# numericalEFT/MCIntegration.jl

Hardware: AMD Instinct MI355X
Metric: Msamples/sec (whole node), 16-D Gaussian :vegas (higher is better)
Workload: dtype f64

## Files before the change

### mcintegration.jl_amd/_lib.py

```python
import ctypes as C
import os

_PKG = os.path.dirname(os.path.abspath(__file__))
_SO = os.path.join(_PKG, "lib", "libmci_hip.so")

MCI_OK = 0
ERR_NAMES = {1: "INVALID", 2: "HIP", 3: "COMPILE", 4: "NORMALIZATION", 5: "HISTOGRAM", 6: "COMM", 7: "NO_DEVICE"}
CONTINUOUS, DISCRETE, FERMIK = 0, 1, 2
VEGAS, VEGASMC, MCMC = 0, 1, 2
ABI_VERSION = 5
SOLVERS = {"vegas": VEGAS, "vegasmc": VEGASMC, "mcmc": MCMC, VEGAS: VEGAS, VEGASMC: VEGASMC, MCMC: MCMC}

c_double_p = C.POINTER(C.c_double)
c_int32_p = C.POINTER(C.c_int32)


class MCIError(RuntimeError):
    def __init__(self, code, msg):
        super().__init__("[MCI_ERR_%s] %s" % (ERR_NAMES.get(code, code), msg))
        self.code = code


class LeafDesc(C.Structure):
    _fields_ = [("kind", C.c_int32), ("pool", C.c_int32), ("lower", C.c_double), ("upper", C.c_double),
# ... 107 lines not shown
    ("mci_last_chain_speculation", C.c_int, [_VP, c_int32_p, c_int32_p]),
    ("mci_chain_speculation_status", C.c_int, [_VP, C.c_int32, c_int32_p]),
    ("mci_vegas_check_status", C.c_int, [_VP, c_int32_p, c_int32_p]),
    ("mci_last_integrate_discarded", C.c_int, [_VP, C.POINTER(C.c_int64), c_int32_p]),
    ("mci_speculation_tree", C.c_int, [C.c_int32, C.c_double, C.c_int32, c_int32_p, c_int32_p, c_int32_p, C.POINTER(C.c_uint64), C.POINTER(C.c_uint64)]),
    ("mci_compile_chain_speculation", C.c_int, [_VP, C.c_int32]),
    ("mci_train", C.c_int, [_VP]),
    ("mci_sample_dump", C.c_int, [_VP, C.c_int32, C.c_uint64, C.c_int64, C.c_int64, C.c_int64, c_double_p, c_double_p, c_double_p]),
    ("mci_kernel_times_ms", C.c_int, [_VP, C.POINTER(C.c_float), C.c_int32, c_int32_p, c_int32_p, c_int32_p]),
    ("mci_kernel_clocks", C.c_int, [_VP, c_double_p, C.c_int32, c_int32_p]),
    ("mci_comm_times_ms", C.c_int, [_VP, C.POINTER(C.c_float), C.c_int32, c_int32_p]),
    ("mci_comm_collectives", C.c_int, [_VP, C.POINTER(C.c_int64), C.POINTER(C.c_int64)]),
    ("mci_reduce_size", C.c_int, [_VP, C.POINTER(C.c_int64)]),
    ("mci_external_reduce_done", C.c_int, [_VP]),
    ("mci_standardize_block", None, [C.c_int64, C.c_int64, C.c_int64, C.POINTER(C.c_int64), C.POINTER(C.c_int64)]),
    ("mci_chain_burnin", C.c_double, [C.c_int64, C.c_int64, C.c_int32]),
    ("mci_mcmc_burnin", C.c_int64, [C.c_int64, C.c_int64, C.c_int32, C.c_int32, C.c_int32, C.c_double]),
    ("mci_mcmc_auto_chains", C.c_int64, [C.c_int64, C.c_int64, C.c_int32, C.c_int32, C.c_int32, C.c_int64, C.c_int64, C.c_int32]),
    ("mci_get_hold_histogram", C.c_int, [_VP, C.POINTER(C.c_uint64)]),
    ("mci_mcmc_launch_valid", C.c_int, [_VP, c_int32_p, c_int32_p, C.POINTER(C.c_int64), C.POINTER(C.c_int64)]),
    ("mci_iteration_discard", C.c_int, [_VP]),
    ("mci_get_block_means", C.c_int, [_VP, C.c_int32, c_double_p, C.POINTER(C.c_int64), c_int32_p]),
    ("mci_reset_block_log", C.c_int, [_VP]),
    ("mci_lineage_sums", None, [c_double_p, C.c_int64, C.c_int64, C.c_int64, c_double_p, C.c_int64, C.c_int64, c_double_p, c_double_p]),
    ("mci_maxdof", None, [c_int32_p, C.c_int32, C.c_int32, c_int32_p]),
    ("mci_mean_std", None, [c_double_p, c_double_p, C.c_int64, C.c_int64, c_double_p, c_double_p]),
    ("mci_average", None, [c_double_p, c_double_p, C.c_int64, C.c_int64, C.c_int64, c_double_p, c_double_p, c_double_p]),
    ("mci_do_reweight", None, [c_double_p, c_double_p, C.c_int64, C.c_double, c_double_p]),
    ("mci_version", C.c_char_p, []),
    ("mci_abi_version", C.c_int32, []),
]
DEBUG_SIGNATURES = [
    ("mci_debug_persist_words", C.c_int, [_VP, C.POINTER(C.c_uint64), C.c_int32]),
    ("mci_debug_walk_counts", C.c_int, [_VP, C.POINTER(C.c_int64)]),
    ("mci_debug_plant_wrong_decision", C.c_int, [_VP, C.c_int32]),
    ("mci_debug_persist_spin_ticks", C.c_int, [_VP, C.c_uint64]),
    ("mci_debug_override", C.c_int, [C.c_char_p, C.c_int64, C.c_int32]),
    ("mci_debug_compiler_id", C.c_int, [C.c_char_p, C.c_char_p, C.c_int32]),
    ("mci_debug_split_chunks", C.c_int, [_VP, C.POINTER(C.c_int64), C.POINTER(C.c_int64)]),
    ("mci_debug_vegas_cursor", C.c_int, [_VP, C.POINTER(C.c_int32), C.POINTER(C.c_uint64)]),
    ("mci_debug_strat_d", C.c_int, [_VP, c_double_p, C.c_int64]),
    ("mci_debug_strat_start_d", C.c_int, [_VP, c_double_p, C.c_int64]),
    ("mci_debug_strat_dump", C.c_int, [_VP, C.c_int64, c_double_p, c_double_p, C.POINTER(C.c_int64), c_double_p, c_double_p]),
    ("mci_debug_mcmc_policy", C.c_int, [C.c_int64, C.c_int64, C.c_int64, C.c_int64]),
    ("mci_debug_vegas_check", C.c_int, [_VP, C.c_int32, C.c_uint64, C.c_int64, C.c_int64, C.c_int64, C.c_int64, c_double_p, c_double_p, c_double_p, c_double_p,
                                        C.POINTER(C.c_int64)]),
    ("mci_debug_vegas_check_launches", C.c_int, [_VP, C.POINTER(C.c_int64)]),
    ("mci_debug_vegas_check_layout", C.c_int, [_VP, c_int32_p, c_int32_p, c_double_p, C.POINTER(C.c_uint64), c_int32_p]),
    ("mci_debug_sweep_workgroups", C.c_int, [_VP, C.c_int32]),
    ("mci_debug_sweep_threads", C.c_int, [_VP, C.c_int32]),
    ("mci_debug_sweep_last_launch", C.c_int, [_VP, c_int32_p, c_int32_p]),
    ("mci_debug_sweep_lds_bytes", C.c_int, [_VP, C.POINTER(C.c_int64)]),
]

_lib = None


def library_path():
    return _SO


def use_rocm_compiler(rocm=None):
    root = rocm or os.environ.get("ROCM_PATH") or "/opt/rocm"
    mapped = set()
    try:
        with open("/proc/self/maps") as fh:
# ... 52 lines not shown
```

### mcintegration.jl_amd/csrc/mci_debug.h

```cpp
#ifndef MCI_DEBUG_H
#define MCI_DEBUG_H
#include "../../include/mci.h"
#ifdef __cplusplus
extern "C" {
#endif
int mci_debug_persist_words(mci_problem *prob, unsigned long long *out, int32_t n);
int mci_debug_walk_counts(mci_problem *prob, int64_t *out);
int mci_debug_plant_wrong_decision(mci_problem *prob, int32_t on);
int mci_debug_persist_spin_ticks(mci_problem *prob, unsigned long long ticks);
int mci_debug_override(const char *key, int64_t value, int32_t on);
int mci_debug_split_chunks(const mci_problem *prob, int64_t *chunks, int64_t *bytes);
int mci_debug_strat_dump(mci_problem *prob, int64_t n, double *x, double *y, int64_t *h, double *jac, double *w);
int mci_debug_strat_d(mci_problem *prob, double *d, int64_t n);
int mci_debug_strat_start_d(mci_problem *prob, double *d, int64_t n);
int mci_debug_vegas_cursor(const mci_problem *prob, int32_t *used, uint64_t *base);
int mci_debug_compiler_id(const char *set, char *out, int32_t n);
int mci_debug_mcmc_policy(int64_t pilot_steps, int64_t grow, int64_t carry_holds, int64_t carry_half_floors);
int mci_debug_vegas_check(mci_problem *prob, int32_t iteration, uint64_t seed, int64_t nevalperblock, int64_t block_lo, int64_t nblocks,
                          int64_t measurefreq, const double *x, const double *jac, const double *w, double *packed, int64_t *bad);
int mci_debug_vegas_check_launches(const mci_problem *prob, int64_t *launches);
int mci_debug_vegas_check_layout(const mci_problem *prob, int32_t *head, int32_t *draws, double *scales, uint64_t *own, int32_t *obs);
int mci_debug_sweep_workgroups(mci_problem *prob, int32_t g);
int mci_debug_sweep_threads(mci_problem *prob, int32_t threads);
int mci_debug_sweep_last_launch(const mci_problem *prob, int32_t *workgroups, int32_t *threads);
int mci_debug_sweep_lds_bytes(const mci_problem *prob, int64_t *bytes);
#ifdef __cplusplus
}
#endif
#endif
```

### mcintegration.jl_amd/csrc/mci_host_jit.h

```cpp
enum { kSlotVegasAny = 3, kSlotDump = 4, kSlotVegasmcSpec = 5, kSlotMcmcSpec = 6 };
static int kslot(int solver, int64_t measurefreq) { return solver == MCI_VEGAS && measurefreq != 1 ? kSlotVegasAny : solver; }
static int slot_solver(int slot) { return slot == kSlotVegasAny ? MCI_VEGAS : slot == kSlotVegasmcSpec ? MCI_VEGASMC : slot == kSlotMcmcSpec ? MCI_MCMC : slot; }

namespace {
struct Candidate {
    std::string src;
    int threads = 256;
    int unit = mcijit::kUnitSolver;
    std::vector<char> code;
    std::string log, path;
    bool cached = false;
    int rc = 0;
    long vgprs() const { return mcijit::kernel_vgprs(code, "mci_vegas_batch"); }
    long scratch() const { return mcijit::kernel_scratch_bytes(code, "mci_vegas_batch"); }
    int build(bool cache_only = false) { return rc = mcijit::compile(src, threads, code, log, cached, &path, unit, cache_only); }
    int failed(const std::string &of = "") const { return fail(MCI_ERR_COMPILE, "integrand failed to compile for gfx950%s:\n%s", of.c_str(), log.c_str()); }
};
void compile_all(const std::vector<Candidate *> &cs) {
    std::vector<std::thread> th;
    for (size_t i = 1; i < cs.size(); ++i) th.emplace_back([c = cs[i]] { c->build(); });
    if (!cs.empty()) cs[0]->build();
    for (auto &t : th) t.join();
}

// ... 484 lines not shown
    return MCI_OK;
}

int mci_set_iteration_counted(mci_problem *p, int32_t counted) {
    if (!p) return fail(MCI_ERR_INVALID, "NULL argument");
    p->launch_counted = counted != 0;
    return MCI_OK;
}

int mci_set_persistent(mci_problem *p, int32_t mode) {
    if (!p) return fail(MCI_ERR_INVALID, "NULL argument");
    if (mode < -1 || mode > 1) return fail(MCI_ERR_INVALID, "persistent mode must be -1 (automatic: launch-bound :vegas calls), 0 (one launch chain per iteration) or 1 (whenever the layout allows)");
    p->persistent = mode;
    return MCI_OK;
}

int mci_debug_persist_words(mci_problem *p, unsigned long long *out, int32_t n) {
    if (!p || !out || !p->d_persist) return fail(MCI_ERR_INVALID, "no persistent launch yet");
    HIPCHK(hipStreamSynchronize(p->ctx->stream));
    HIPCHK(hipMemcpy(out, p->d_persist, (size_t)(n < (int)kPersistWords ? n : (int)kPersistWords) * sizeof(unsigned long long), hipMemcpyDeviceToHost));
    return MCI_OK;
}

int mci_debug_walk_counts(mci_problem *p, int64_t *out) {
    if (!p || !out || !p->d_status) return fail(MCI_ERR_INVALID, "NULL argument");
    int h[2] = {0, 0};
    HIPCHK(hipStreamSynchronize(p->ctx->stream));
    HIPCHK(hipMemcpy(h, p->d_status + 1, sizeof(h), hipMemcpyDeviceToHost));
    out[0] = h[0];
    out[1] = h[1];
    return MCI_OK;
}

int mci_last_integrate_persistent(const mci_problem *p, int32_t *persistent) {
    if (!p || !persistent) return fail(MCI_ERR_INVALID, "NULL argument");
    *persistent = p->last_persistent ? 1 : 0;
    return MCI_OK;
}

int mci_last_chain_launch(const mci_problem *p, int64_t *nchain, int32_t *carried) {
    if (!p) return fail(MCI_ERR_INVALID, "NULL argument");
    if (nchain) *nchain = p->launch.last_nchain;
    if (carried) *carried = p->launch.last_carried ? 1 : 0;
    return MCI_OK;
}

int mci_check_status(mci_problem *p) {
    if (!p) return fail(MCI_ERR_INVALID, "NULL argument");
    if (p->ctx->offline) return fail(MCI_ERR_NO_DEVICE, "offline context");
    return check_status(p);
}
static int compile_persist(mci_problem *p, bool background);
static bool persist_layout_ok(const mci_problem *p);
static int compile_strat(mci_problem *p);
static int compile_sweep_unit(mci_problem *p, int which);
static bool sweep_leaves_unit(const mci_problem *p);
int mci_compile_solver(mci_problem *p, int32_t solver) {
    if (solver == MCI_VEGAS_PERSISTENT) {
        if (!persist_layout_ok(p)) return fail(MCI_ERR_INVALID, "this layout has no persistent :vegas kernel (mci_set_persistent)");
        return compile_persist(p, false);
    }
    if (solver == MCI_VEGASMC_LANES || solver == MCI_MCMC_LANES) return mci_compile_chain_speculation(p, solver == MCI_VEGASMC_LANES ? MCI_VEGASMC : MCI_MCMC);
    if (solver == MCI_VEGAS_STRAT) {
        if (!p->strat.on) return fail(MCI_ERR_INVALID, "the problem is not stratified (mci_set_stratification)");
        return compile_strat(p);
    }
// ... 51 lines not shown
```

### mcintegration.jl_amd/csrc/mci_host_problem.h

```cpp
int mci_problem_create(mci_ctx *ctx, const mci_problem_desc *d, mci_problem **out) {
    if (!ctx || !d || !out) return fail(MCI_ERR_INVALID, "NULL argument");
    if (d->nleaf < 1 || d->npool < 1 || d->nintegrand < 1) return fail(MCI_ERR_INVALID, "At least one integrand is required.");
    if (d->nintegrand > 31) return fail(MCI_ERR_INVALID, "at most 31 integrands are supported");
    mci_problem *p = new mci_problem();
    p->ctx = ctx;
    p->npool = d->npool;
    p->ni = d->nintegrand;
    const int Nd = p->ni + 1;
    p->dof.assign((size_t)Nd * p->npool, 0);
    for (int i = 0; i < p->ni * p->npool; ++i) {
        if (d->dof[i] < 0) { delete p; return fail(MCI_ERR_INVALID, "dof must be non-negative"); }
        p->dof[i] = d->dof[i];
    }
    p->maxdof.assign(p->npool, 0);
    mci_maxdof(p->dof.data(), Nd, p->npool, p->maxdof.data());
    p->pool_leaf0.assign(p->npool, -1);
    p->pool_nleaf.assign(p->npool, 0);
    auto &s = p->shape;
    int eoff = 0, aoff = 0, doff = 0, boff = 0;
    for (int l = 0; l < d->nleaf; ++l) {
        const mci_leaf_desc &ld = d->leaves[l];
        if (ld.pool < 0 || ld.pool >= p->npool) { delete p; return fail(MCI_ERR_INVALID, "leaf %d: pool out of range", l); }
        if (p->pool_leaf0[ld.pool] < 0) p->pool_leaf0[ld.pool] = l;
        else if (p->pool_leaf0[ld.pool] + p->pool_nleaf[ld.pool] != l) { delete p; return fail(MCI_ERR_INVALID, "leaves of pool %d are not contiguous", ld.pool); }
// ... 264 lines not shown
            if (g_over.hist_copies.on) {
                hc = (int)g_over.hist_copies.v;
                while (hc > 1 && (!hist_lds || s.ntile != 1 || (hc & (hc - 1)) || p->lds_bytes + one * (hc - 1) > lim1)) hc >>= 1;
                if (hc < 1) hc = 1;
            }
            s.hcopy = hc;
        }
        const int64_t hcopy_bytes = (int64_t)s.htile * 8 * (s.hcopy - 1);
        if (mode == 3 && s.ntile == 1) {
            const int64_t budget = (lim1 - p->lds_bytes - hcopy_bytes) / 8;
            for (size_t l = 0; l < p->leaves.size(); ++l) {
                const Leaf &L = p->leaves[l];
                if (L.kind != MCI_CONTINUOUS || s.ec_doubles + L.nbin + 1 > budget) continue;
                s.leaf_ecoff[l] = s.ec_doubles;
                s.ec_doubles += L.nbin + 1;
            }
            p->lds_bytes_k1 = p->lds_bytes + (int64_t)s.ec_doubles * 8;
        }
        s.l1_phase = (mode == 3 && s.split_all) ? 1 : 0;
        if (g_over.l1_phase.on) s.l1_phase = (mode >= 2 && g_over.l1_phase.v > 0) ? 1 : 0;
        if (p->lds_bytes > lim0) p->threads = 512;
        p->vegas.created(s.hcopy, p->lds_bytes > lim0);
    }
    p->nstat = 2 * s.nobs + 2 + Nd;
    p->packed_n = p->nstat + s.nbin + 2 * p->npa;
    p->h_reweight.assign(Nd, 1.0 / Nd);
    s.body = "w[0] = 1.0;";
    if (!ctx->offline) {
        HIPCHK(hipSetDevice(ctx->device));
        int rc = upload(p);
        if (!rc) rc = p->d_packed.reserve(p->packed_n + 64);
        if (!rc) rc = p->d_ghist.reserve(3 * (int64_t)(s.nbin ? s.nbin : 1));
        if (!rc) rc = p->d_stage1.reserve((int64_t)mci_problem::kGroups * (s.nbin ? s.nbin : 1));
        if (!rc) rc = p->d_status.reserve(4);
        std::vector<mci::LeafDev> ld;
        for (auto &L : p->leaves) ld.push_back({L.kind, L.nbin, L.eoff, L.doff, L.boff, L.adapt, L.alpha});
        if (!rc) rc = p->d_leaves.reserve((int64_t)ld.size());
        if (rc) { delete p; return rc; }
        HIPCHK(hipMemset(p->d_packed, 0, (size_t)(p->packed_n + 64) * sizeof(double)));
        HIPCHK(hipMemset(p->d_ghist, 0, 3 * (size_t)(s.nbin ? s.nbin : 1) * sizeof(double)));
        HIPCHK(hipMemset(p->d_status, 0, 4 * sizeof(int)));
        HIPCHK(hipMemcpy(p->d_leaves, ld.data(), ld.size() * sizeof(mci::LeafDev), hipMemcpyHostToDevice));
        p->evs.resize(2 * mci_problem::kEvRing);
        for (auto &e : p->evs) HIPCHK(hipEventCreate(&e));
    }
    *out = p;
    return MCI_OK;
}

int mci_problem_destroy(mci_problem *p) {
    if (!p) return MCI_OK;
    if (!p->ctx->offline) {
        (void)hipStreamSynchronize(p->ctx->stream);
        for (KernelUnit &u : p->kernel) u.drop();
    }
    persist_job_drop(p);
    if (!p->ctx->offline) {
        if (p->hold_ev) (void)hipEventDestroy(p->hold_ev);
        for (auto &e : p->cevs) (void)hipEventDestroy(e);
        tile_release(p);
        for (auto &e : p->evs) (void)hipEventDestroy(e);
    }
    delete p;
    return MCI_OK;
}

int mci_set_integrand_source(mci_problem *p, const char *body, const double *ud, int32_t nud) {
    if (!p || !body) return fail(MCI_ERR_INVALID, "NULL argument");
    p->shape.body = body;
    p->shape.host_integrand = 0;
    p->host_fn = nullptr;
    p->h_ud.assign(ud, ud + (nud > 0 ? nud : 0));
    drop_modules(p);
    if (!p->ctx->offline) {
// ... 157 lines not shown
```

### mcintegration.jl_amd/csrc/mci_host_types.h

```cpp
namespace {

struct Id128 { char b[128]; };
struct Rccl {
    void *h = nullptr;
    int (*GetUniqueId)(void *) = nullptr;
    int (*CommInitRank)(void **, int, Id128 , int) = nullptr;
    int (*AllReduce)(const void *, void *, size_t, int, int, void *, hipStream_t) = nullptr;
    int (*CommDestroy)(void *) = nullptr;
    const char *(*GetErrorString)(int) = nullptr;
};
Rccl g_rccl;
const int kNcclFloat64 = 8, kNcclSum = 0;

int find_loaded_rccl(struct dl_phdr_info *info, size_t, void *out) {
    const char *n = info->dlpi_name;
    if (n && strstr(n, "librccl.so")) {
        *(std::string *)out = n;
        return 1;
    }
    return 0;
}

int rccl_load() {
    if (g_rccl.h) return MCI_OK;
// ... 321 lines not shown
static const int kRepeatStride = 16384, kMaxRepeats = 7;

int64_t mci_problem::kMcmcPilotSteps = 4096;
int64_t mci_problem::kMcmcGrow = 2;
int64_t mci_problem::kMcmcCarryHolds = 4;
int64_t mci_problem::kMcmcCarryHalfFloors = 2;

namespace {
struct Override { bool on = false; int64_t v = 0; };
struct Overrides { Override table_mode, hist_tile_bins, no_split_all, l1_phase, train_walk, hist_copies, fresh_floors, fresh_burnin_pct, spec_self_check, split_chunk, vegas_self_check, vegas_cursor, cursor_log2_big, cursor_ones; } g_over;
Override *override_slot(const char *key) {
    if (!key) return nullptr;
    if (!strcmp(key, "table_mode")) return &g_over.table_mode;
    if (!strcmp(key, "hist_tile_bins")) return &g_over.hist_tile_bins;
    if (!strcmp(key, "no_split_all")) return &g_over.no_split_all;
    if (!strcmp(key, "l1_phase")) return &g_over.l1_phase;
    if (!strcmp(key, "train_walk")) return &g_over.train_walk;
    if (!strcmp(key, "hist_copies")) return &g_over.hist_copies;
    if (!strcmp(key, "fresh_floors")) return &g_over.fresh_floors;
    if (!strcmp(key, "fresh_burnin_pct")) return &g_over.fresh_burnin_pct;
    if (!strcmp(key, "spec_self_check")) return &g_over.spec_self_check;
    if (!strcmp(key, "split_chunk")) return &g_over.split_chunk;
    if (!strcmp(key, "vegas_self_check")) return &g_over.vegas_self_check;
    if (!strcmp(key, "vegas_cursor")) return &g_over.vegas_cursor;
    if (!strcmp(key, "cursor_log2_big")) return &g_over.cursor_log2_big;
    if (!strcmp(key, "cursor_ones")) return &g_over.cursor_ones;
    return nullptr;
}
}

static void persist_job_drop(mci_problem *p);
namespace { void persist_orphans_join(); }
static const size_t kPersistWords = 8 + 3 * 8 * 8 + 16;

namespace {

int tile_alloc(mci_problem *p, size_t bytes) {
    mci_ctx *c = p->ctx;
    void *base = nullptr;
    {
        std::lock_guard<std::mutex> g(c->spare_mu);
        if (c->spare && c->spare_bytes >= bytes && c->spare_bytes <= 2 * bytes + ((size_t)64 << 20)) {
            base = c->spare;
            p->tile_bytes = c->spare_bytes;
            c->spare = nullptr;
            c->spare_bytes = 0;
        }
    }
    if (!base) {
        HIPCHK(hipMalloc(&base, bytes));
        p->tile_bytes = bytes;
    }
    p->d_tile_w = (double *)base;
    return MCI_OK;
}
void tile_release(mci_problem *p) {
    if (!p->d_tile_w) return;
    mci_ctx *c = p->ctx;
    void *drop = p->d_tile_w;
    {
        std::lock_guard<std::mutex> g(c->spare_mu);
        if (p->tile_bytes > c->spare_bytes) {
            drop = c->spare;
            c->spare = p->d_tile_w;
            c->spare_bytes = p->tile_bytes;
        }
// ... 201 lines not shown
```

### mcintegration.jl_amd/csrc/mci_static_kernels.h

```cpp
#pragma once
#include <hip/hip_runtime.h>

#include "mci_train.h"
#include "mci_strat.h"

namespace mci {

__global__ void __launch_bounds__(256) k_hist_stage1(const double *__restrict__ part_hist, int nwg, int nbin, int ngroup,
                                                     double *__restrict__ out) {
    const int bin = blockIdx.x * 256 + threadIdx.x;
    const int g = blockIdx.y;
    if (bin >= nbin) return;
    const int per = (nwg + ngroup - 1) / ngroup;
    const int w0 = g * per, w1 = min(nwg, w0 + per);
    double s0 = 0.0, s1 = 0.0, s2 = 0.0, s3 = 0.0;
    int w = w0;
    for (; w + 3 < w1; w += 4) {
        s0 += part_hist[(size_t)(w + 0) * nbin + bin];
        s1 += part_hist[(size_t)(w + 1) * nbin + bin];
        s2 += part_hist[(size_t)(w + 2) * nbin + bin];
        s3 += part_hist[(size_t)(w + 3) * nbin + bin];
    }
    for (; w < w1; ++w) s0 += part_hist[(size_t)w * nbin + bin];
    out[(size_t)g * nbin + bin] = (s0 + s1) + (s2 + s3);
}

__global__ void __launch_bounds__(256) k_add_host_obs(const double *__restrict__ obs, int nblocks, int nobs, int ncols, int wg_per_block,
                                                      double *__restrict__ part_cols) {
    const int i = blockIdx.x * 256 + threadIdx.x;
    if (i >= nblocks * nobs) return;
    const int b = i / nobs, o = i % nobs;
    part_cols[(size_t)b * wg_per_block * ncols + o] += obs[i];
}

__global__ void __launch_bounds__(256) k_finalize(MergeArgs m) {
    const int nhb = (m.nbin + 255) / 256;
    const int hoff = 2 * m.nobs + 2 + m.ni + 1;
    if ((int)blockIdx.x < nhb) {
        const int bin = blockIdx.x * 256 + threadIdx.x;
        if (bin < m.nbin) m.packed[hoff + bin] = merge_hist_bin(m, bin);
        return;
    }
    if ((int)blockIdx.x > nhb) {
        merge_pa(m, (int)blockIdx.x - nhb - 1);
        return;
    }
    merge_stats(m);
}

struct ResampleArgs {
    const int *curr_old;
    long long n_old, n_new;
    int nd;
    const double *rw_now, *rw_used;
    int *src;
    double *W;
    const double *w_chain;
// ... 86 lines not shown
    const double step = W[a.n_old - 1] / (double)a.n_new;
    if (!(W[a.n_old - 1] > 0.0)) {
        for (long long c = tid; c < a.n_new; c += T) src[c] = (int)(c % a.n_old);
        return;
    }
    for (long long c = tid; c < a.n_new; c += T) {
        const double target = ((double)c + 0.6180339887498949) * step;
        long long lo = 0, hi = a.n_old - 1;
        while (lo < hi) {
            const long long mid = (lo + hi) >> 1;
            if ((in_lds ? sW[mid] : W[mid]) > target) hi = mid;
            else lo = mid + 1;
        }
        src[c] = (int)lo;
    }
}

__global__ void __launch_bounds__(512) k_train(TrainArgs a) {
    extern __shared__ __attribute__((aligned(16))) double sm[];
    __shared__ double ps[256];
    __shared__ int bad;
    __shared__ double ssum;
    if ((int)blockIdx.x == a.nleaf) {
        iteration_bookkeeping(a);
        return;
    }
    if (!a.do_train) return;
    const LeafDev L = a.leaves[blockIdx.x];
    if (!L.adapt) return;
    double *h = a.packed + a.nstat + L.boff;
    train_leaf(L, h, h, sm, ps, bad, ssum, a.edges, a.dacc, a.ddist, a.serial_walk, a.status, false, nullptr, false, a.spare ? sm + train_lds_doubles(a.maxn) : nullptr);
}

__global__ void __launch_bounds__(512) k_finish(MergeArgs m, TrainArgs a) {
    extern __shared__ __attribute__((aligned(16))) double sm[];
    __shared__ double ps[256];
    __shared__ int bad;
    __shared__ double ssum;
    const int tid = threadIdx.x, T = blockDim.x;
    if ((int)blockIdx.x == a.nleaf) {
        merge_stats(m);
        __syncthreads();
        iteration_bookkeeping(a);
        return;
    }
    if ((int)blockIdx.x > a.nleaf) {
        merge_pa(m, (int)blockIdx.x - a.nleaf - 1);
        return;
    }
    const LeafDev L = a.leaves[blockIdx.x];
    double *hl = sm + train_lds_doubles(a.maxn);
    double *hp = a.packed + a.nstat + L.boff;
    const bool train = a.do_train && L.adapt;
    if (train) train_stage_grid(L, sm, a.edges);
    for (int i = tid; i < L.nbin; i += T) {
        const double v = merge_hist_bin(m, L.boff + i);
        hl[i] = v;
        hp[i] = v;
    }
    __syncthreads();
    if (!train) return;
    train_leaf(L, hl, hp, sm, ps, bad, ssum, a.edges, a.dacc, a.ddist, a.serial_walk, a.status, true, nullptr, false, a.spare ? hl : nullptr);
}

struct StratAllocArgs {
    const double *d;
    long long *off;
    double *tsum;
    long long ncube, nsamp;
    int ntile;
    int uniform;
};
__global__ void __launch_bounds__(256) k_strat_alloc(StratAllocArgs a, int phase) {
    __shared__ double part[256];
    const int tid = threadIdx.x;
    if (phase == 1) {
        if (tid != 0) return;
        double base = 0.0;
        for (int g = 0; g < a.ntile; ++g) {
            a.tsum[a.ntile + g] = base;
            base += a.tsum[g];
        }
        a.tsum[2 * a.ntile] = base;
        a.tsum[2 * a.ntile + 1] = strat_alloc_uniform(a.uniform, base) ? 1.0 : 0.0;
        return;
    }
    long long lo, hi;
    strat_alloc_stretch(a.ncube, a.ntile, (int)blockIdx.x, tid, lo, hi);
    const bool uniform = phase == 2 && a.tsum[2 * a.ntile + 1] != 0.0;
    part[tid] = uniform ? 0.0 : strat_alloc_stretch_sum(a.d, lo, hi);
    __syncthreads();
    if (phase == 0) {
        if (tid == 0) a.tsum[blockIdx.x] = strat_alloc_base(part, 256);
        return;
    }
// ... 109 lines not shown
```

### mcintegration.jl_amd/csrc/mci_train.h

```cpp
#pragma once
#include "mci_device.h"

namespace mci {


struct LeafDev {
    int kind;
    int nbin;
    int eoff;
    int doff;
    int boff;
    int adapt;
    double alpha;
};


enum { kMergeGroups = 32 };

struct MergeArgs {
    const double *part_cols;
    int ncols, nobs, ni, nblocks, wg_per_block;
    const double *stage1;
    int ngroup;
    double *ghist;
// ... 123 lines not shown
    double base = 0.0;
    for (int w = 0; w < wave; ++w) base += ps[w];
    (void)nwave;
    double run = base + (x - loc);
    for (int k = b; k < e; ++k) {
        run += v[k];
        out[k] = run;
    }
    __syncthreads();
    return out[n - 1];
}

enum { kWalkPad = 64 };
__host__ __device__ inline int train_lds_doubles(int n) { return (n + kWalkPad) + (n + 2) + (n + kWalkPad) + 2; }
__host__ __device__ inline int train_spare_doubles(int n) { return 2 * (2 * n + kWalkPad) + (2 * n + kWalkPad) / 16 + 2; }

__device__ inline double sum16(const double *v, int n) {
    double s = 0.0;
    int i = threadIdx.x & 15;
    for (; i + 496 < n; i += 512) {
        double t[32];
#pragma unroll
        for (int k = 0; k < 32; ++k) t[k] = v[i + 16 * k];
#pragma unroll
        for (int k = 0; k < 32; ++k) s += t[k];
    }
    for (; i + 112 < n; i += 128) {
        double t[8];
#pragma unroll
        for (int k = 0; k < 8; ++k) t[k] = v[i + 16 * k];
#pragma unroll
        for (int k = 0; k < 8; ++k) s += t[k];
    }
    for (; i < n; i += 16) s += v[i];
    s += dpp_read<0x108, 0xf>(s);
    s += dpp_read<0x104, 0xf>(s);
    s += dpp_read<0x102, 0xf>(s);
    s += dpp_read<0x101, 0xf>(s);
    return __shfl(s, 0, 16);
}

#ifdef MCI_TRAIN_SHORT_SUMS
template <int DEPTH = 3> __device__ inline double sum_julia(const double *v, int n) { return sum16(v, n); }
#else
template <int DEPTH = 3> __device__ inline double sum_julia(const double *v, int n) {
    if constexpr (DEPTH == 0) return sum16(v, n);
    else {
        if (n <= 1024) return sum16(v, n);
        const int h = ((n - 1) >> 1) + 1;
        return sum_julia<DEPTH - 1>(v, h) + sum_julia<DEPTH - 1>(v + h, n - h);
    }
}
#endif

__device__ inline double rescale_pow(double b, double alpha) {
    if (alpha == 2.0) return b * b;
    if (alpha == 1.0) return b;
    if (alpha == 3.0) return b * b * b;
    return pow(b, alpha);
}

struct TrainArgs {
    const LeafDev *leaves;
    int nleaf;
    double *packed;
    int nstat;
    double *edges, *dacc, *ddist;
// ... 49 lines not shown
                 MCI_WALK_MORE("9", "%15")
                 MCI_WALK_MORE("10", "%16")
                 MCI_WALK_MORE("11", "%17")
                 MCI_WALK_MORE("12", "%18")
                 MCI_WALK_MORE("13", "%19")
                 MCI_WALK_MORE("14", "%20")
                 MCI_WALK_MORE("15", "%21")
                 ".Lwend_%=:"
                 : "+v"(acc), "=&v"(a1), "=&s"(c2)
                 : "v"(f), "v"(rec_addr), "v"(v[0]), "v"(v[1]), "v"(v[2]), "v"(v[3]), "v"(v[4]), "v"(v[5]), "v"(v[6]), "v"(v[7]), "v"(v[8]),
                   "v"(v[9]), "v"(v[10]), "v"(v[11]), "v"(v[12]), "v"(v[13]), "v"(v[14]), "v"(v[15]), "v"(vnext)
                 : "vcc", "scc", "memory");
}

#undef MCI_WALK_BIN
#undef MCI_WALK_MORE

template <bool RECORD> __device__ __forceinline__ void walk_slots16(double &acc, const double (&e)[16], double *__restrict__ rec) {
    if (!RECORD) rec[0] = acc;
#pragma unroll
    for (int k = 0; k < 16; ++k) {
        if (RECORD) rec[k] = acc;
        acc = acc + e[k];
    }
}

__device__ __forceinline__ void walk_trip(double &acc, const double (&v)[16], const double vnext, const double f, const unsigned rec_addr) {
    walk_bins16(acc, v, vnext, f, rec_addr);
}
#endif

enum { kTrainQ = 4 };

__device__ inline void train_stage_grid(const LeafDev &L, double *sm, const double *__restrict__ edges) {
    if (L.kind != 0) return;
    const int tid = threadIdx.x, T = blockDim.x, N = L.nbin;
    double *d = sm, *sg = sm + N + kWalkPad;
    const double *g = edges + L.eoff;
    for (int base = 0; base <= N; base += kTrainQ * T) {
        double v[kTrainQ];
#pragma unroll
        for (int q = 0; q < kTrainQ; ++q) {
            const int i = base + q * T + tid;
            v[q] = i <= N ? g[i] : 0.0;
        }
#pragma unroll
        for (int q = 0; q < kTrainQ; ++q) {
            const int i = base + q * T + tid;
            if (i <= N) sg[i] = v[q];
        }
    }
    if (tid < kWalkPad) d[N + tid] = 0.0;
}

__device__ inline void train_leaf(const LeafDev &L, const double *h, double *hclear, double *sm, double *ps, int &bad, double &ssum,
                                  double *__restrict__ edges, double *__restrict__ dacc, double *__restrict__ ddist, int serial_walk,
                                  int *__restrict__ status, bool staged = false, unsigned long long *tt = nullptr, bool checked = false,
                                  double *spare = nullptr) {
#ifdef MCI_PERSIST_TRACE
#define MCI_TT(k) if (tt && threadIdx.x == 0) tt[k] = wall_clock64();
#else
#define MCI_TT(k)
    (void)tt;
#endif
    const int tid = threadIdx.x, T = blockDim.x;
    const int N = L.nbin;
    double *d = sm;
    double *sg = sm + N + kWalkPad;
    double *wa = sg + N + 2;
    MCI_TT(0)
    if (!checked) {
        if (tid == 0) bad = 0;
        __syncthreads();
        for (int i = tid; i < N; i += T) {
            const double v = h[i];
            if (!isfinite(v)) atomicOr(&bad, ST_HIST_NONFINITE);
            else if (!(v > 0.0)) atomicOr(&bad, ST_HIST_NONPOSITIVE);
        }
        __syncthreads();
    }
    if (bad) {
        if (tid == 0) atomicOr(status, bad);
        return;
    }
    if (L.kind == 0) {
        double *g = edges + L.eoff;
        MCI_TT(1)
        if (!staged) train_stage_grid(L, sm, edges);
        double mine = 0.0;
        for (int i = tid; i < N; i += T) {
            double v;
            if (N <= 1) v = h[i];
            else if (i == 0) v = (h[0] * 7.0 + h[1]) / 8.0;
            else if (i == N - 1) v = (h[N - 1] * 7.0 + h[N - 2]) / 8.0;
            else v = (h[i - 1] + h[i] * 6.0 + h[i + 1]) / 8.0;
            d[i] = v;
            mine += v;
        }
        if (!serial_walk) {
            const double w = wave_sum(mine);
            if ((tid & 63) == 0) ps[32 + (tid >> 6)] = w;
        }
        __syncthreads();
        MCI_TT(2)
        if (N > 1) {
            double s;
            if (serial_walk) {
                s = sum_julia(d, N);
                __syncthreads();
            } else {
                s = 0.0;
                for (int w = 0; w < (T >> 6); ++w) s += ps[32 + w];
            }
            MCI_TT(3)
            int anybad = 0;
            auto rescale_q = [&](auto power, auto QC) {
                constexpr int Q = decltype(QC)::value;
                for (int base = 0; base < N; base += Q * T) {
                    double v[Q];
#pragma unroll
                    for (int q = 0; q < Q; ++q) {
                        const int i = base + q * T + tid;
                        v[q] = i < N ? d[i] / s : 1.0;
                    }
#pragma unroll
                    for (int q = 0; q < Q; ++q) {
                        const double r = power(-(1 - v[q]) / log(v[q]));
                        v[q] = (v[q] > 0 && v[q] <= 0.99999999) ? r : v[q];
                    }
#pragma unroll
                    for (int q = 0; q < Q; ++q) {
                        const int i = base + q * T + tid;
                        if (!isfinite(v[q])) anybad = 1;
                        if (i < N) d[i] = v[q];
                    }
                }
            };
            auto rescale_bins = [&](auto power) {
#ifdef MCI_TRAIN_SCAN_ONLY
                rescale_q(power, IC<(MCI_THREADS >= 512 ? 2 : kTrainQ)>{});
#else
                if (2 * T >= N) rescale_q(power, IC<2>{});
// ... 47 lines not shown
                    for (int q = 0; q < Q; ++q) {
                        lo[q] += wa[lo[q]] < target[q] ? 1 : 0;
                        lo[q] = lo[q] > N - 1 ? N - 1 : lo[q];
                    }
                    double vnew[Q];
#pragma unroll
                    for (int q = 0; q < Q; ++q) {
                        const int i = base + q * T + tid, j = lo[q];
                        const double acc_f = wa[j] - target[q];
                        const double v = sg[j + 1] - (acc_f / d[j]) * (sg[j + 1] - sg[j]);
                        vnew[q] = (i == 0 || i >= N) ? sg[i < N ? 0 : N] : v;
                    }
#pragma unroll
                    for (int q = 0; q < Q; ++q) {
                        const int i = base + q * T + tid;
                        if (i <= N) g[i] = vnew[q];
                    }
                }
            };
#ifdef MCI_TRAIN_SCAN_ONLY
            place_points(IC<(MCI_THREADS >= 512 ? 2 : kTrainQ)>{});
#else
            if (2 * T > N) place_points(IC<2>{});
            else place_points(IC<kTrainQ>{});
#endif
            __syncthreads();
            MCI_TT(6)
            if (hclear)
                for (int i = tid; i < N; i += T) hclear[i] = 1.0e-10;
            MCI_TT(7)
            return;
        }
#ifndef MCI_TRAIN_SCAN_ONLY
        const double f_ninc = sum_julia(d, N) / (double)N;
        if (!(f_ninc > 0.0 && isfinite(f_ninc))) {
            if (tid == 0) atomicOr(status, ST_RESCALE_NONFINITE);
            return;
        }
        int *flag = (int *)(ps + 64);
        int *pw = (int *)ps;
        const int lane = tid & 63, wave = tid >> 6;
        const int per = (N + T - 1) / T, b = min(N, tid * per), e = min(N, b + per);
        bool given = spare != nullptr && serial_walk != 2 && N > 1;
        double *es = spare, *rs = spare + 2 * N + kWalkPad, *heads = rs + 2 * N + kWalkPad;
        const double f_inv = 1.0 / f_ninc, f_lo = 0.5 * f_ninc, f_hi = 2.0 * f_ninc;
        auto points = [&](int j) {
            if (j >= N - 1) return 0;
            const double c = floor(wa[j] * f_inv) - (j > 0 ? floor(wa[j - 1] * f_inv) : 0.0);
            if (serial_walk == 3 && j == N / 2) return c > 0.0 ? (int)c + 1 : 1;
            return c > 0.0 ? (int)c : 0;
        };
        auto slots = [&](int j, int c) { return c + ((c >= 1 && d[j + 1] >= f_lo && d[j + 1] <= f_hi) ? 0 : 1); };
        int sbase = 0, nslot = 0;
        if (given) {
            if (tid == 0) *flag = 0;
            block_prefix(d, wa, N, ps);
            int mine = 0;
            for (int j = b; j < e; ++j) mine += slots(j, points(j));
            int x = mine;
#pragma unroll
            for (int off = 1; off < 64; off <<= 1) {
                const int y = __shfl_up(x, off, 64);
                if (lane >= off) x += y;
            }
            if (lane == 63) pw[wave] = x;
            __syncthreads();
            for (int w = 0; w < (T >> 6); ++w) {
                if (w < wave) sbase += pw[w];
                nslot += pw[w];
            }
            sbase += x - mine;
            int sl = sbase;
            for (int j = b; j < e; ++j) {
                const int c = points(j);
                for (int k = 0; k < c - 1; ++k) es[sl++] = -f_ninc;
                if (c >= 1 && slots(j, c) == c) es[sl++] = d[j + 1] - f_ninc;
                else {
                    if (c >= 1) es[sl++] = -f_ninc;
                    es[sl++] = d[j + 1];
                }
            }
            for (int k = nslot + tid; k < nslot + kWalkPad; k += T) es[k] = 0.0;
            __syncthreads();
        }
        int cnt;
        for (;;) {
            if (tid == 0) {
                double va[16], vb[16];
                double acc_f = 0.0 + d[0];
                if (given) {
#pragma unroll
                    for (int k = 0; k < 16; ++k) va[k] = es[k];
                    for (int sb = 0; sb < nslot; sb += 32) {
#pragma unroll
                        for (int k = 0; k < 16; ++k) vb[k] = es[sb + 16 + k];
                        walk_slots16<false>(acc_f, va, heads + (sb >> 4));
#pragma unroll
                        for (int k = 0; k < 16; ++k) va[k] = es[sb + 32 + k];
                        walk_slots16<false>(acc_f, vb, heads + (sb >> 4) + 1);
                    }
                } else {
                    const unsigned rec = (unsigned)(size_t)wa;
#pragma unroll
                    for (int k = 0; k < 16; ++k) va[k] = d[k];
                    for (int jb = 0; jb < N; jb += 32) {
#pragma unroll
                        for (int k = 0; k < 16; ++k) vb[k] = d[jb + 16 + k];
                        walk_trip(acc_f, va, vb[0], f_ninc, rec + 8u * (unsigned)jb);
#pragma unroll
                        for (int k = 0; k < 16; ++k) va[k] = d[jb + 32 + k];
                        walk_trip(acc_f, vb, va[0], f_ninc, rec + 8u * (unsigned)(jb + 16));
                    }
                }
            }
            __syncthreads();
            if (given) {
                for (int t = tid; t * 16 < nslot; t += T) {
                    double ev[16];
#pragma unroll
                    for (int k = 0; k < 16; ++k) ev[k] = es[t * 16 + k];
                    double acc_f = heads[t];
                    walk_slots16<true>(acc_f, ev, rs + t * 16);
                }
                __syncthreads();
            }
            cnt = 0;
            int wrong = 0, sl = sbase;
            for (int j = b; j < e; ++j) {
                int c = 0;
                for (double a = given ? rs[sl] : wa[j]; a >= f_ninc; a -= f_ninc) c += 1;
                cnt += c;
                if (given) {
                    const int cp = points(j);
                    wrong |= (j < N - 1 && c != cp) ? 1 : 0;
                    sl += slots(j, cp);
                }
            }
            if (!given) break;
            if (wrong) atomicOr(flag, 1);
            __syncthreads();
            if (*flag == 0) break;
            given = false;
        }
        if (tid == 0) atomicAdd(status + (given ? 1 : 2), 1);
        {
            int x = cnt;
#pragma unroll
            for (int off = 1; off < 64; off <<= 1) {
                const int y = __shfl_up(x, off, 64);
                if (lane >= off) x += y;
            }
            if (lane == 63) pw[wave] = x;
            __syncthreads();
            int base = 0, total = 0;
            for (int w = 0; w < (T >> 6); ++w) {
                if (w < wave) base += pw[w];
                total += pw[w];
            }
            int i = 1 + base + x - cnt;
            int sl = sbase;
            for (int j = b; j < e; ++j) {
                for (double a = given ? rs[sl] : wa[j]; a >= f_ninc;) {
                    a -= f_ninc;
                    if (i < N) g[i] = sg[j + 1] - (a / d[j]) * (sg[j + 1] - sg[j]);
                    i += 1;
                }
                if (given) sl += slots(j, points(j));
            }
            for (int k = 1 + total + tid; k < N; k += T) g[k] = sg[N];
            if (tid == 0) {
                g[0] = sg[0];
                g[N] = sg[N];
            }
        }
#endif
    }
#ifndef MCI_TRAIN_CONTINUOUS_ONLY
    else {
        double *acc = dacc + L.eoff, *dist = ddist + L.doff;
        const double s = N > 1 ? sum_julia(h, N) : 1.0;
        if (tid == 0) {
            int lbad = 0;
            if (N > 1) {
                for (int i = 0; i < N; ++i) {
                    double v = h[i] / s;
                    if (v > 0 && v <= 0.99999999) v = rescale_pow(-(1 - v) / log(v), L.alpha);
                    if (!isfinite(v)) lbad = ST_RESCALE_NONFINITE;
                    d[i] = v;
                }
            } else {
                d[0] = h[0];
            }
            if (lbad) {
                atomicOr(status, lbad);
            } else {
                double s = 0.0;
                for (int i = 0; i < N; ++i) s += d[i];
                double run = 0.0;
                acc[0] = 0.0;
                for (int i = 0; i < N; ++i) {
                    const double v = d[i] / s;
                    dist[i] = v;
                    run += v;
                    acc[i + 1] = run;
                }
            }
        }
    }
#endif
    __syncthreads();
    if (hclear)
        for (int i = tid; i < N; i += T) hclear[i] = 1.0e-10;
#undef MCI_TT
}

__device__ inline void iteration_bookkeeping(const TrainArgs &a) {
    const int tid = threadIdx.x, T = blockDim.x;
    double *row = a.iter_log_row;
    if (row)
        for (int i = tid; i < a.nstat; i += T) row[i] = a.packed[i];
#ifndef MCI_TRAIN_CONTINUOUS_ONLY
    if (a.do_reweight && tid == 0) do_reweight_dev(a.reweight, a.packed + (a.nstat - a.nd), a.nd, a.gamma, a.goal);
#endif
}

struct PersistArgs {
    MergeArgs m;
    TrainArgs t;
    int niter;
    int map_off;
    u64 *ctr;
    u64 arrive0, done0;
    u64 spin_ticks;
};

enum : u64 { kPersistDoneShift = 40, kPersistArriveMask = (1ull << 40) - 1 };
__device__ __forceinline__ bool persist_wait(const PersistArgs &f, u64 t0, u64 t1, int *verdict) {
    if (threadIdx.x == 0) {
        int ok = 1;
        const u64 start = wall_clock64();
        unsigned n = 0;
        for (;;) {
            const u64 w = __hip_atomic_load(&f.ctr[0], __ATOMIC_RELAXED, __HIP_MEMORY_SCOPE_AGENT);
            if ((w & kPersistArriveMask) >= t0 && (long long)(((w >> kPersistDoneShift) - t1) << kPersistDoneShift) >= 0) break;
            __builtin_amdgcn_s_sleep(1);
// ... 140 lines not shown
```

Baseline: 76240.

## Speed up finish kernel training walk with register-held bins and DPP scans

Restructures the grid-training step in the finish kernel. Each thread now keeps its per-bin counts, slots and neighbour values in registers when it owns at most kTrainQ bins, the shuffle-based integer prefix scan is replaced by a DPP scan, and the normalization sum runs on one wave and overlaps with the block prefix. The histogram clear is moved earlier, a redundant barrier is skipped by clearing the bad flag up front, and the stage-1 histogram reduction issues up to 16 loads at once. It also adds optional wall-clock tracing and a debug readout for it. This aims to cut serial latency in the per-iteration training tail, at the cost of more registers and more code paths.

```diff
diff --git a/mcintegration.jl_amd/_lib.py b/mcintegration.jl_amd/_lib.py
--- a/mcintegration.jl_amd/_lib.py
+++ b/mcintegration.jl_amd/_lib.py
@@ -163,6 +163,7 @@
 ]
 DEBUG_SIGNATURES = [
     ("mci_debug_persist_words", C.c_int, [_VP, C.POINTER(C.c_uint64), C.c_int32]),
+    ("mci_debug_finish_stamps", C.c_int, [_VP, C.POINTER(C.c_uint64), C.c_int32]),
     ("mci_debug_walk_counts", C.c_int, [_VP, C.POINTER(C.c_int64)]),
     ("mci_debug_plant_wrong_decision", C.c_int, [_VP, C.c_int32]),
     ("mci_debug_persist_spin_ticks", C.c_int, [_VP, C.c_uint64]),
diff --git a/mcintegration.jl_amd/csrc/mci_debug.h b/mcintegration.jl_amd/csrc/mci_debug.h
--- a/mcintegration.jl_amd/csrc/mci_debug.h
+++ b/mcintegration.jl_amd/csrc/mci_debug.h
@@ -5,6 +5,7 @@
 extern "C" {
 #endif
 int mci_debug_persist_words(mci_problem *prob, unsigned long long *out, int32_t n);
+int mci_debug_finish_stamps(mci_problem *prob, unsigned long long *out, int32_t n);
 int mci_debug_walk_counts(mci_problem *prob, int64_t *out);
 int mci_debug_plant_wrong_decision(mci_problem *prob, int32_t on);
 int mci_debug_persist_spin_ticks(mci_problem *prob, unsigned long long ticks);
diff --git a/mcintegration.jl_amd/csrc/mci_host_jit.h b/mcintegration.jl_amd/csrc/mci_host_jit.h
--- a/mcintegration.jl_amd/csrc/mci_host_jit.h
+++ b/mcintegration.jl_amd/csrc/mci_host_jit.h
@@ -540,6 +540,19 @@
     return MCI_OK;
 }
 
+int mci_debug_finish_stamps(mci_problem *p, unsigned long long *out, int32_t n) {
+    if (!p || !out || !p->d_status) return fail(MCI_ERR_INVALID, "NULL argument");
+#ifdef MCI_FINISH_TRACE
+    if (n > (int32_t)mci::kFinishStamps) n = (int32_t)mci::kFinishStamps;
+    HIPCHK(hipStreamSynchronize(p->ctx->stream));
+    HIPCHK(hipMemcpy(out, p->d_status + 4, (size_t)n * sizeof(unsigned long long), hipMemcpyDeviceToHost));
+    return MCI_OK;
+#else
+    (void)n;
+    return fail(MCI_ERR_INVALID, "this library was built without -DMCI_FINISH_TRACE (tools/finish_trace.py builds one that has it)");
+#endif
+}
+
 int mci_last_integrate_persistent(const mci_problem *p, int32_t *persistent) {
     if (!p || !persistent) return fail(MCI_ERR_INVALID, "NULL argument");
     *persistent = p->last_persistent ? 1 : 0;
diff --git a/mcintegration.jl_amd/csrc/mci_host_problem.h b/mcintegration.jl_amd/csrc/mci_host_problem.h
--- a/mcintegration.jl_amd/csrc/mci_host_problem.h
+++ b/mcintegration.jl_amd/csrc/mci_host_problem.h
@@ -320,14 +320,14 @@
         if (!rc) rc = p->d_packed.reserve(p->packed_n + 64);
         if (!rc) rc = p->d_ghist.reserve(3 * (int64_t)(s.nbin ? s.nbin : 1));
         if (!rc) rc = p->d_stage1.reserve((int64_t)mci_problem::kGroups * (s.nbin ? s.nbin : 1));
-        if (!rc) rc = p->d_status.reserve(4);
+        if (!rc) rc = p->d_status.reserve(kStatusWords);
         std::vector<mci::LeafDev> ld;
         for (auto &L : p->leaves) ld.push_back({L.kind, L.nbin, L.eoff, L.doff, L.boff, L.adapt, L.alpha});
         if (!rc) rc = p->d_leaves.reserve((int64_t)ld.size());
         if (rc) { delete p; return rc; }
         HIPCHK(hipMemset(p->d_packed, 0, (size_t)(p->packed_n + 64) * sizeof(double)));
         HIPCHK(hipMemset(p->d_ghist, 0, 3 * (size_t)(s.nbin ? s.nbin : 1) * sizeof(double)));
-        HIPCHK(hipMemset(p->d_status, 0, 4 * sizeof(int)));
+        HIPCHK(hipMemset(p->d_status, 0, kStatusWords * sizeof(int)));
         HIPCHK(hipMemcpy(p->d_leaves, ld.data(), ld.size() * sizeof(mci::LeafDev), hipMemcpyHostToDevice));
         p->evs.resize(2 * mci_problem::kEvRing);
         for (auto &e : p->evs) HIPCHK(hipEventCreate(&e));
diff --git a/mcintegration.jl_amd/csrc/mci_host_types.h b/mcintegration.jl_amd/csrc/mci_host_types.h
--- a/mcintegration.jl_amd/csrc/mci_host_types.h
+++ b/mcintegration.jl_amd/csrc/mci_host_types.h
@@ -377,6 +377,11 @@
 static void persist_job_drop(mci_problem *p);
 namespace { void persist_orphans_join(); }
 static const size_t kPersistWords = 8 + 3 * 8 * 8 + 16;
+#ifdef MCI_FINISH_TRACE
+static const size_t kStatusWords = 4 + 2 * mci::kFinishStamps;
+#else
+static const size_t kStatusWords = 4;
+#endif
 
 namespace {
 
diff --git a/mcintegration.jl_amd/csrc/mci_static_kernels.h b/mcintegration.jl_amd/csrc/mci_static_kernels.h
--- a/mcintegration.jl_amd/csrc/mci_static_kernels.h
+++ b/mcintegration.jl_amd/csrc/mci_static_kernels.h
@@ -6,14 +6,32 @@
 
 namespace mci {
 
-__global__ void __launch_bounds__(256) k_hist_stage1(const double *__restrict__ part_hist, int nwg, int nbin, int ngroup,
-                                                     double *__restrict__ out) {
-    const int bin = blockIdx.x * 256 + threadIdx.x;
-    const int g = blockIdx.y;
-    if (bin >= nbin) return;
+enum { kStage1Flight = 16 };
+__host__ __device__ inline void stage1_group_rows(int nwg, int ngroup, int g, int &w0, int &w1) {
     const int per = (nwg + ngroup - 1) / ngroup;
-    const int w0 = g * per, w1 = min(nwg, w0 + per);
+    w0 = g * per;
+    w1 = w0 + per < nwg ? w0 + per : nwg;
+}
+__host__ __device__ inline double stage1_sum(const double *__restrict__ part_hist, int w0, int w1, int nbin, int bin) {
     double s0 = 0.0, s1 = 0.0, s2 = 0.0, s3 = 0.0;
+    const int n = w1 - w0;
+    if (n > 0 && n <= kStage1Flight) {
+        double v[kStage1Flight];
+#pragma unroll
+        for (int k = 0; k < kStage1Flight; ++k) v[k] = k < n ? part_hist[(size_t)(w0 + k) * nbin + bin] : 0.0;
+#pragma unroll
+        for (int k = 0; k < kStage1Flight; k += 4)
+            if (k + 3 < n) {
+                s0 += v[k + 0];
+                s1 += v[k + 1];
+                s2 += v[k + 2];
+                s3 += v[k + 3];
+            }
+#pragma unroll
+        for (int k = 0; k < kStage1Flight; ++k)
+            if (k >= (n & ~3) && k < n) s0 += v[k];
+        return (s0 + s1) + (s2 + s3);
+    }
     int w = w0;
     for (; w + 3 < w1; w += 4) {
         s0 += part_hist[(size_t)(w + 0) * nbin + bin];
@@ -22,7 +40,17 @@
         s3 += part_hist[(size_t)(w + 3) * nbin + bin];
     }
     for (; w < w1; ++w) s0 += part_hist[(size_t)w * nbin + bin];
-    out[(size_t)g * nbin + bin] = (s0 + s1) + (s2 + s3);
+    return (s0 + s1) + (s2 + s3);
+}
+
+__global__ void __launch_bounds__(256) k_hist_stage1(const double *__restrict__ part_hist, int nwg, int nbin, int ngroup,
+                                                     double *__restrict__ out) {
+    const int bin = blockIdx.x * 256 + threadIdx.x;
+    const int g = blockIdx.y;
+    if (bin >= nbin) return;
+    int w0, w1;
+    stage1_group_rows(nwg, ngroup, g, w0, w1);
+    out[(size_t)g * nbin + bin] = stage1_sum(part_hist, w0, w1, nbin, bin);
 }
 
 __global__ void __launch_bounds__(256) k_add_host_obs(const double *__restrict__ obs, int nblocks, int nobs, int ncols, int wg_per_block,
@@ -175,12 +203,22 @@
     train_leaf(L, h, h, sm, ps, bad, ssum, a.edges, a.dacc, a.ddist, a.serial_walk, a.status, false, nullptr, false, a.spare ? sm + train_lds_doubles(a.maxn) : nullptr);
 }
 
+enum { kFinishStamps = 24 };
 __global__ void __launch_bounds__(512) k_finish(MergeArgs m, TrainArgs a) {
     extern __shared__ __attribute__((aligned(16))) double sm[];
     __shared__ double ps[256];
     __shared__ int bad;
     __shared__ double ssum;
     const int tid = threadIdx.x, T = blockDim.x;
+#ifdef MCI_FINISH_TRACE
+    __shared__ unsigned long long ttl[kFinishStamps];
+    unsigned long long *tt = blockIdx.x == 0 ? ttl : nullptr;
+    if (tt && tid < kFinishStamps) tt[tid] = 0ull;
+    __syncthreads();
+    if (tt && tid == 0) tt[18] = wall_clock64();
+#else
+    unsigned long long *tt = nullptr;
+#endif
     if ((int)blockIdx.x == a.nleaf) {
         merge_stats(m);
         __syncthreads();
@@ -195,6 +233,7 @@
     double *hl = sm + train_lds_doubles(a.maxn);
     double *hp = a.packed + a.nstat + L.boff;
     const bool train = a.do_train && L.adapt;
+    if (tid == 0) bad = 0;
     if (train) train_stage_grid(L, sm, a.edges);
     for (int i = tid; i < L.nbin; i += T) {
         const double v = merge_hist_bin(m, L.boff + i);
@@ -203,7 +242,11 @@
     }
     __syncthreads();
     if (!train) return;
-    train_leaf(L, hl, hp, sm, ps, bad, ssum, a.edges, a.dacc, a.ddist, a.serial_walk, a.status, true, nullptr, false, a.spare ? hl : nullptr);
+    train_leaf(L, hl, hp, sm, ps, bad, ssum, a.edges, a.dacc, a.ddist, a.serial_walk, a.status, true, tt, false, a.spare ? hl : nullptr, true);
+#ifdef MCI_FINISH_TRACE
+    __syncthreads();
+    if (tt && tid < kFinishStamps) reinterpret_cast<unsigned long long *>(a.status + 4)[tid] = tt[tid];
+#endif
 }
 
 struct StratAllocArgs {
diff --git a/mcintegration.jl_amd/csrc/mci_train.h b/mcintegration.jl_amd/csrc/mci_train.h
--- a/mcintegration.jl_amd/csrc/mci_train.h
+++ b/mcintegration.jl_amd/csrc/mci_train.h
@@ -179,7 +179,14 @@
 #pragma unroll
         for (int k = 0; k < 8; ++k) s += t[k];
     }
-    for (; i < n; i += 16) s += v[i];
+    {
+        double t[8];
+#pragma unroll
+        for (int k = 0; k < 8; ++k) t[k] = i + 16 * k < n ? v[i + 16 * k] : 0.0;
+#pragma unroll
+        for (int k = 0; k < 8; ++k)
+            if (i + 16 * k < n) s += t[k];
+    }
     s += dpp_read<0x108, 0xf>(s);
     s += dpp_read<0x104, 0xf>(s);
     s += dpp_read<0x102, 0xf>(s);
@@ -295,6 +302,19 @@
 
 enum { kTrainQ = 4 };
 
+template <int CTRL, int ROW_MASK> __device__ __forceinline__ int dpp_read_i(int v) {
+    return __builtin_amdgcn_update_dpp(0, v, CTRL, ROW_MASK, 0xf, false);
+}
+__device__ __forceinline__ int wave_scan_incl_i(int v) {
+    v += dpp_read_i<0x111, 0xf>(v);
+    v += dpp_read_i<0x112, 0xf>(v);
+    v += dpp_read_i<0x114, 0xf>(v);
+    v += dpp_read_i<0x118, 0xf>(v);
+    v += dpp_read_i<0x142, 0xa>(v);
+    v += dpp_read_i<0x143, 0xc>(v);
+    return v;
+}
+
 __device__ inline void train_stage_grid(const LeafDev &L, double *sm, const double *__restrict__ edges) {
     if (L.kind != 0) return;
     const int tid = threadIdx.x, T = blockDim.x, N = L.nbin;
@@ -319,8 +339,8 @@
 __device__ inline void train_leaf(const LeafDev &L, const double *h, double *hclear, double *sm, double *ps, int &bad, double &ssum,
                                   double *__restrict__ edges, double *__restrict__ dacc, double *__restrict__ ddist, int serial_walk,
                                   int *__restrict__ status, bool staged = false, unsigned long long *tt = nullptr, bool checked = false,
-                                  double *spare = nullptr) {
-#ifdef MCI_PERSIST_TRACE
+                                  double *spare = nullptr, bool bad_cleared = false) {
+#if defined(MCI_PERSIST_TRACE) || defined(MCI_FINISH_TRACE)
 #define MCI_TT(k) if (tt && threadIdx.x == 0) tt[k] = wall_clock64();
 #else
 #define MCI_TT(k)
@@ -333,8 +353,10 @@
     double *wa = sg + N + 2;
     MCI_TT(0)
     if (!checked) {
-        if (tid == 0) bad = 0;
-        __syncthreads();
+        if (!bad_cleared) {
+            if (tid == 0) bad = 0;
+            __syncthreads();
+        }
         for (int i = tid; i < N; i += T) {
             const double v = h[i];
             if (!isfinite(v)) atomicOr(&bad, ST_HIST_NONFINITE);
@@ -369,8 +391,12 @@
         if (N > 1) {
             double s;
             if (serial_walk) {
-                s = sum_julia(d, N);
+                if (tid < 64) {
+                    const double t = sum_julia(d, N);
+                    if (tid == 0) ssum = t;
+                }
                 __syncthreads();
+                s = ssum;
             } else {
                 s = 0.0;
                 for (int w = 0; w < (T >> 6); ++w) s += ps[32 + w];
@@ -484,17 +510,28 @@
             return;
         }
 #ifndef MCI_TRAIN_SCAN_ONLY
-        const double f_ninc = sum_julia(d, N) / (double)N;
-        if (!(f_ninc > 0.0 && isfinite(f_ninc))) {
-            if (tid == 0) atomicOr(status, ST_RESCALE_NONFINITE);
-            return;
-        }
+        if (tid < 64) {
+            const double t = sum_julia(d, N);
+            if (tid == 0) ssum = t;
+        }
+        MCI_TT(8)
         int *flag = (int *)(ps + 64);
         int *pw = (int *)ps;
         const int lane = tid & 63, wave = tid >> 6;
         const int per = (N + T - 1) / T, b = min(N, tid * per), e = min(N, b + per);
         bool given = spare != nullptr && serial_walk != 2 && N > 1;
         double *es = spare, *rs = spare + 2 * N + kWalkPad, *heads = rs + 2 * N + kWalkPad;
+        if (given) {
+            if (tid == 0) *flag = 0;
+            block_prefix(d, wa, N, ps);
+        } else
+            __syncthreads();
+        MCI_TT(9)
+        const double f_ninc = ssum / (double)N;
+        if (!(f_ninc > 0.0 && isfinite(f_ninc))) {
+            if (tid == 0) atomicOr(status, ST_RESCALE_NONFINITE);
+            return;
+        }
         const double f_inv = 1.0 / f_ninc, f_lo = 0.5 * f_ninc, f_hi = 2.0 * f_ninc;
         auto points = [&](int j) {
             if (j >= N - 1) return 0;
@@ -504,17 +541,47 @@
         };
         auto slots = [&](int j, int c) { return c + ((c >= 1 && d[j + 1] >= f_lo && d[j + 1] <= f_hi) ? 0 : 1); };
         int sbase = 0, nslot = 0;
+        const bool inreg = per <= kTrainQ;
+        int cq[kTrainQ], sq[kTrainQ];
+        double dn[kTrainQ];
+#pragma unroll
+        for (int q = 0; q < kTrainQ; ++q) {
+            cq[q] = 0;
+            sq[q] = 0;
+            dn[q] = 0.0;
+        }
         if (given) {
-            if (tid == 0) *flag = 0;
-            block_prefix(d, wa, N, ps);
             int mine = 0;
+            if (inreg) {
+                double fl[kTrainQ + 1];
+                fl[0] = (b > 0 && b < e) ? wa[b - 1] : 0.0;
+#pragma unroll
+                for (int q = 0; q < kTrainQ; ++q) {
+                    const int j = b + q;
+                    fl[q + 1] = j < e ? wa[j] : 0.0;
+                    dn[q] = j < e ? d[j + 1] : 0.0;
+                }
+                fl[0] = b > 0 ? floor(fl[0] * f_inv) : 0.0;
+#pragma unroll
+                for (int q = 0; q < kTrainQ; ++q) fl[q + 1] = floor(fl[q + 1] * f_inv);
+#pragma unroll
+                for (int q = 0; q < kTrainQ; ++q) {
+                    const int j = b + q;
+                    if (j < e) {
+                        int c = 0;
+                        if (j < N - 1) {
+                            const double cd = fl[q + 1] - fl[q];
+                            if (serial_walk == 3 && j == N / 2) c = cd > 0.0 ? (int)cd + 1 : 1;
+                            else c = cd > 0.0 ? (int)cd : 0;
+                        }
+                        cq[q] = c;
+                        sq[q] = c + ((c >= 1 && dn[q] >= f_lo && dn[q] <= f_hi) ? 0 : 1);
+                        mine += sq[q];
+                    }
+                }
+            } else
             for (int j = b; j < e; ++j) mine += slots(j, points(j));
-            int x = mine;
-#pragma unroll
-            for (int off = 1; off < 64; off <<= 1) {
-                const int y = __shfl_up(x, off, 64);
-                if (lane >= off) x += y;
-            }
+            const int x = wave_scan_incl_i(mine);
             if (lane == 63) pw[wave] = x;
             __syncthreads();
             for (int w = 0; w < (T >> 6); ++w) {
@@ -522,7 +589,22 @@
                 nslot += pw[w];
             }
             sbase += x - mine;
+            MCI_TT(10)
             int sl = sbase;
+            if (inreg) {
+#pragma unroll
+                for (int q = 0; q < kTrainQ; ++q) {
+                    if (b + q < e) {
+                        const int c = cq[q];
+                        for (int k = 0; k < c - 1; ++k) es[sl++] = -f_ninc;
+                        if (c >= 1 && sq[q] == c) es[sl++] = dn[q] - f_ninc;
+                        else {
+                            if (c >= 1) es[sl++] = -f_ninc;
+                            es[sl++] = dn[q];
+                        }
+                    }
+                }
+            } else
             for (int j = b; j < e; ++j) {
                 const int c = points(j);
                 for (int k = 0; k < c - 1; ++k) es[sl++] = -f_ninc;
@@ -534,7 +616,19 @@
             }
             for (int k = nslot + tid; k < nslot + kWalkPad; k += T) es[k] = 0.0;
             __syncthreads();
-        }
+            MCI_TT(11)
+        }
+        if (hclear)
+            for (int i = tid; i < N; i += T) hclear[i] = 1.0e-10;
+        hclear = nullptr;
+        double sgq[kTrainQ + 1], dq[kTrainQ], aq[kTrainQ];
+#pragma unroll
+        for (int q = 0; q < kTrainQ; ++q) {
+            dq[q] = (inreg && b + q < e) ? d[b + q] : 1.0;
+            aq[q] = 0.0;
+        }
+#pragma unroll
+        for (int q = 0; q <= kTrainQ; ++q) sgq[q] = (inreg && b < e && b + q <= e) ? sg[b + q] : 0.0;
         int cnt;
         for (;;) {
             if (tid == 0) {
@@ -566,6 +660,7 @@
                 }
             }
             __syncthreads();
+            MCI_TT(12)
             if (given) {
                 for (int t = tid; t * 16 < nslot; t += T) {
                     double ev[16];
@@ -575,9 +670,26 @@
                     walk_slots16<true>(acc_f, ev, rs + t * 16);
                 }
                 __syncthreads();
+                MCI_TT(13)
             }
             cnt = 0;
             int wrong = 0, sl = sbase;
+            if (inreg) {
+#pragma unroll
+                for (int q = 0; q < kTrainQ; ++q) {
+                    if (b + q < e) aq[q] = given ? rs[sl] : wa[b + q];
+                    sl += sq[q];
+                }
+#pragma unroll
+                for (int q = 0; q < kTrainQ; ++q) {
+                    if (b + q < e) {
+                        int c = 0;
+                        for (double a = aq[q]; a >= f_ninc; a -= f_ninc) c += 1;
+                        cnt += c;
+                        if (given) wrong |= (b + q < N - 1 && c != cq[q]) ? 1 : 0;
+                    }
+                }
+            } else
             for (int j = b; j < e; ++j) {
                 int c = 0;
                 for (double a = given ? rs[sl] : wa[j]; a >= f_ninc; a -= f_ninc) c += 1;
@@ -594,14 +706,10 @@
             if (*flag == 0) break;
             given = false;
         }
+        MCI_TT(14)
         if (tid == 0) atomicAdd(status + (given ? 1 : 2), 1);
         {
-            int x = cnt;
-#pragma unroll
-            for (int off = 1; off < 64; off <<= 1) {
-                const int y = __shfl_up(x, off, 64);
-                if (lane >= off) x += y;
-            }
+            const int x = wave_scan_incl_i(cnt);
             if (lane == 63) pw[wave] = x;
             __syncthreads();
             int base = 0, total = 0;
@@ -609,8 +717,20 @@
                 if (w < wave) base += pw[w];
                 total += pw[w];
             }
+            MCI_TT(15)
             int i = 1 + base + x - cnt;
             int sl = sbase;
+            if (inreg) {
+#pragma unroll
+                for (int q = 0; q < kTrainQ; ++q) {
+                    if (b + q < e)
+                        for (double a = aq[q]; a >= f_ninc;) {
+                            a -= f_ninc;
+                            if (i < N) g[i] = sgq[q + 1] - (a / dq[q]) * (sgq[q + 1] - sgq[q]);
+                            i += 1;
+                        }
+                }
+            } else
             for (int j = b; j < e; ++j) {
                 for (double a = given ? rs[sl] : wa[j]; a >= f_ninc;) {
                     a -= f_ninc;
@@ -624,6 +744,7 @@
                 g[0] = sg[0];
                 g[N] = sg[N];
             }
+            MCI_TT(16)
         }
 #endif
     }
@@ -663,6 +784,7 @@
     __syncthreads();
     if (hclear)
         for (int i = tid; i < N; i += T) hclear[i] = 1.0e-10;
+    MCI_TT(17)
 #undef MCI_TT
 }
 
```

Measured after the change: 76360, median of 5. About the same (+0.2%).
